# Gabrielcb/DaliID

Hardware: AMD Instinct MI355X
Metric: images/sec (train step) (higher is better)
Workload: dtype bf16; 1 GPU; configs[1]: ResNet-50 ReID bf16 256x128, PK batch 16x16=256 per GPU, center+proxy heads, Adam, EMA; global_batch=256, per_gpu_batch=256, parallelism=dp1

## Files before the change

daliid_amd/csrc/conv.hip:

```cpp
#include "gemm_tile.h"
#include "kernels.h"
#include "../../include/daliid_debug.h"
#include <cstdlib>
#include <type_traits>
#include <vector>
#include <string>
#include <cstdio>

namespace dali {

__device__ __forceinline__ void decode_pixel(const GatherGeom& g, int p, int& n, int& ho, int& wo) {
    if (g.lhw >= 0 && g.lw >= 0) {
        n = p >> g.lhw;
        const int rem = p & ((1 << g.lhw) - 1);
        ho = rem >> g.lw;
        wo = rem & ((1 << g.lw) - 1);
    } else {
        const int hw = g.Hout * g.Wout;
        n = p / hw;
        const int rem = p - n * hw;
        ho = rem / g.Wout;
        wo = rem - ho * g.Wout;
    }
}
// ... 1336 lines not shown
        if (ksteps > 1) dma_wait<4>(); else dma_wait<0>();
        __builtin_amdgcn_s_barrier();
        conv_stamp(a, 1);
        int st_cur = 0, st_nxt2 = 2;
        for (int kt = 0; kt < ksteps; ++kt) {
            if (kt + 2 < ksteps) issue(kt + 2, st_nxt2);
            const uint16_t* sa = smem + st_cur * 2 * TILE;
            const uint16_t* sb = sa + TILE;
            bf16x8_t fa[4];
            wgrad_tr_kstep(sa, wm * 4, sb, wn * 4, lane, acc, fa);
            if constexpr (COLSUM) if (do_cs) {
#pragma unroll
                for (int i = 0; i < 4; ++i) cs[i] = __builtin_amdgcn_mfma_f32_16x16x32_bf16(fa[i], ones, cs[i], 0, 0, 0);
            }
            if (kt + 2 < ksteps) dma_wait<4>(); else dma_wait<0>();
            __builtin_amdgcn_s_barrier();
            st_cur = (st_cur == 2) ? 0 : st_cur + 1;
            st_nxt2 = (st_nxt2 == 2) ? 0 : st_nxt2 + 1;
        }
    }
    conv_stamp(a, 2);
    float* slab = a.partial + (size_t)ks * a.Cm * a.Ntot;
    store_slab_tiles<4, 4>(slab, acc, m0 + wm * 64, n0 + wn * 64, a.Cm, a.Ntot, lane);
    if constexpr (COLSUM) if (do_cs && (lane & 15) == 0) {
#pragma unroll
        for (int i = 0; i < 4; ++i)
#pragma unroll
            for (int rr = 0; rr < 4; ++rr) {
                const int m = m0 + wm * 64 + i * 16 + (lane >> 4) * 4 + rr;
                if (m < a.Cm) a.colsum[(size_t)ks * a.Cm + m] = cs[i][rr];
            }
    }
    conv_stamp_stores(a);
}

__device__ __forceinline__ int halo_swz(int row) { return ((row >> 1) & 1) | (((row >> 3) & 1) << 1); }
constexpr int W3_A_ELEMS = 32 * 128, W3_B_ELEMS = 16 * 512, W3_STAGE = W3_A_ELEMS + W3_B_ELEMS;

template <int NSTAGE>
__global__ __launch_bounds__(512) void igemm_wgrad3x3_kernel(WGradArgs a, int tiles_m, int tiles_n) {
    extern __shared__ __attribute__((aligned(16))) uint16_t smem[];
    const int tid = threadIdx.x, lane = tid & 63;
    const int wave = __builtin_amdgcn_readfirstlane(tid >> 6);
    const int wm = wave >> 2, wn = wave & 3;
    WGradWork wk;
    if (!wk.map_xcd(a, tiles_m, tiles_n)) return;
    const int ks = wk.ks, m0 = wk.tm * 128, ci0 = wk.tn * 64;
    conv_stamp(a, 0);
    const bool m_active = m0 + wm * 64 < a.Cm;
    const GatherGeom g = a.g;
    const int W = g.Wout, H = g.Hout, Cin = g.Ck, lw = g.lw, lhw = g.lhw;
    const int RW = 32 >> lw, HC = W + 2, HP = (RW + 2) * HC;
    const WGradRsrc rs = wgrad_rsrc(a);

    const int r_in = lane >> 4, ps = lane & 15;
    const int c16 = ((((ps >> 1) ^ wg_swz(4 * wave + r_in)) << 1) | (ps & 1));
    const int am = m0 + c16 * 8;
    const bool a_ok = am < a.Cm;
    int hb_hr[2], hb_off[2];
    bool hb_ok[2];
#pragma unroll
    for (int i = 0; i < 2; ++i) {
        const int hp = 8 * (wave + 8 * i) + (lane >> 3);
        const int lc = (lane & 7) ^ (halo_swz(hp) << 1);
        const int hr = hp / HC, hc = hp - hr * HC;
        hb_hr[i] = hr;
// ... 562 lines not shown
    K64_CLS = ring_kernel<64, 4, 4, 4, 4, 2, 4, true, Epi::PARITY>("K64_CLS"),
    K64_SRC2 = ring_kernel<64, 4, 4, 4, 4, 2, 4, true, Epi::CONV, true>("K64_SRC2"),
    K64_FUSED_SRC2 = ring_kernel<64, 4, 4, 4, 4, 2, 4, true, Epi::FUSED, true>("K64_FUSED_SRC2"),
    K64_320 = ring_kernel<64, 4, 4, 4, 5, 2, 4, true, Epi::LIN>("K64_320");

template <int RB, bool RES, bool OM, bool BITS, bool SRC2 = false>
static GemmKernel f1_kernel() {
    static char name[32];
    snprintf(name, sizeof name, "F1_RB%d%s%s%s%s", RB, RES ? "_RES" : "", OM ? "_MASK" : "", BITS ? "_BITS" : "", SRC2 ? "_SRC2" : "");
    return {name, kfn(&fused1x1_persist_kernel<3, RB, RES, OM, BITS, SRC2>), (F1_NC + F1_NP + F1_NR) * 64, f1_lds_bytes(3, RB, RB == 2 ? 128 : F1_KMAX),
            F1_TM, F1_TN, GRID_CUS, 0, RB};
}
static const GemmKernel F1[2][2][2][2] = {
    {{{f1_kernel<2, false, false, false, true>(), f1_kernel<2, false, false, true>()}, {f1_kernel<2, false, true, false>(), f1_kernel<2, false, true, true>()}},
     {{f1_kernel<2, true, false, false>(), f1_kernel<2, true, false, true>()}, {f1_kernel<2, true, true, false>(), f1_kernel<2, true, true, true>()}}},
    {{{f1_kernel<1, false, false, false, true>(), f1_kernel<1, false, false, true>()}, {f1_kernel<1, false, true, false>(), f1_kernel<1, false, true, true>()}},
     {{f1_kernel<1, true, false, false>(), f1_kernel<1, true, false, true>()}, {f1_kernel<1, true, true, false>(), f1_kernel<1, true, true, true>()}}}};

static const GemmKernel
    WG_BN{"WG_BN", kfn(&igemm_wgrad_kernel<true>), 256, 0, 128, 128, GRID_SPLITS},
    WG_PLAIN{"WG_PLAIN", kfn(&igemm_wgrad_kernel<false>), 256, 0, 128, 128, GRID_SPLITS},
    WG_3X3{"WG_3X3", kfn(&igemm_wgrad3x3_kernel<3>), 512, 3 * W3_STAGE * 2, 128, 9 * 64, GRID_SPLITS8, 256};
static const GemmKernel WG_DMA[2] = {
    {"WG_DMA", kfn(&igemm_wgrad_dma_kernel<false>), 256, 0, 128, 128, GRID_SPLITS8},
    {"WG_DMA_COLSUM", kfn(&igemm_wgrad_dma_kernel<true>), 256, 0, 128, 128, GRID_SPLITS8}};
static const GemmKernel WG_WG[2] = {
    {"WG_WG", kfn(&igemm_wgrad_wg_kernel<2, 4, 3>), 512, ring_lds(128, 256, 32, 3), 128, 256, GRID_SPLITS8, 512},
    {"WG_WG_COLSUM", kfn(&igemm_wgrad_wg_kernel<2, 4, 3, true>), 512, ring_lds(128, 256, 32, 3), 128, 256, GRID_SPLITS8, 512}};
static const GemmKernel WG_P[2][2] = {
    {{"WG_P", kfn(&igemm_wgrad_p_kernel<2, 4, 4, 4, 8, 6>), 1024, ring_lds(128, 256, 32, 6), 128, 256, GRID_SPLITS8, 256},
     {"WG_P_COLSUM", kfn(&igemm_wgrad_p_kernel<2, 4, 4, 4, 8, 6, true>), 1024, ring_lds(128, 256, 32, 6), 128, 256, GRID_SPLITS8, 256}},
    {{"WG_P_FLAT", kfn(&igemm_wgrad_p_kernel<1, 4, 8, 4, 4, 6>), 512, ring_lds(128, 256, 32, 6), 128, 256, GRID_SPLITS8, 256},
     {"WG_P_FLAT_COLSUM", kfn(&igemm_wgrad_p_kernel<1, 4, 8, 4, 4, 6, true>), 512, ring_lds(128, 256, 32, 6), 128, 256, GRID_SPLITS8, 256}}};

struct GemmChoice {
    const GemmKernel* k = nullptr;
    int tiles_m = 0, tiles_n = 0, lds = 0, class_grid = 0;
    unsigned grid = 0;
    int rc = DALI_OK, why_arg = 0;
    const char* why = nullptr;
    GemmChoice() = default;
    GemmChoice(int rc_, const char* why_, int why_arg_ = 0) : rc(rc_), why_arg(why_arg_), why(why_) {}
    int refuse() const { set_error(why, why_arg); return rc; }
};
static GemmChoice gemm_place(const GemmKernel& k, int rows, int cols, int mult, int Ck) {
    GemmChoice c;
    c.k = &k;
    c.tiles_m = (rows + k.tm - 1) / k.tm;
    c.tiles_n = (cols + k.tn - 1) / k.tn;
    c.lds = k.f1_rb ? f1_lds_bytes(3, k.f1_rb, Ck) : k.lds;
    switch (k.grid) {
        case GRID_XCD: c.grid = xcd_tile_grid(c.tiles_m, c.tiles_n); break;
        case GRID_CLASSES: c.class_grid = xcd_tile_grid(c.tiles_m, c.tiles_n); c.grid = mult * c.class_grid; break;
        case GRID_CUS: c.grid = mult; break;
        case GRID_HALO: c.grid = c.tiles_n; break;
        case GRID_SPLITS: c.grid = c.tiles_m * c.tiles_n * mult; break;
        case GRID_SPLITS8: c.grid = (c.tiles_m * c.tiles_n * mult + 7) / 8 * 8; break;
    }
    return c;
}
template <class Args>
static int gemm_launch(hipStream_t st, const GemmChoice& c, Args& args) {
    const GemmKernel& k = *c.k;
    DeviceOnce::Guard once(k.once);
    if (k.lds > 64 * 1024 && once.first()) {
        DALI_HIP(hipFuncSetAttribute(k.fn, hipFuncAttributeMaxDynamicSharedMemorySize, k.lds));
// ... 232 lines not shown
    wgrad_plan(Cm, w.Ntot, P, 512, &w.splits, &w.pix_per_split, taps, halo_w);
    const int cfg = wgrad_pick_cfg(Cm, w.Ntot, taps, P, halo_w);
    const bool dma_ok = gather_dma_ok(g, P, (long long)P * Cm * 2);
    const bool colsum = want_colsum && wgrad_colsum_ok(cfg, in_bn, dma_ok);
    w.c = gemm_place(wgrad_kernel(cfg, Cm, w.Ntot, in_bn, dma_ok, colsum, plain_rows(g)), Cm, w.Ntot, w.splits, g.Ck);
    w.colsum_rows = colsum ? colsum_rows_of(*w.c.k, w.Ntot, w.splits) : 0;
    return w;
}

WGradNeed wgrad_need(int Cm, int P, const GatherGeom& g, bool colsum, bool operand_transform) {
    const WGradChoice w = wgrad_choose(Cm, P, g, operand_transform, colsum);
    return WGradNeed{(size_t)w.splits * Cm * w.Ntot * sizeof(float), colsum ? std::max((size_t)w.colsum_rows * Cm, colsum_partial_floats(P, Cm)) : 0};
}

int launch_wgrad(hipStream_t st, WGradArgs a, const WGradBufs& ws, float* out, int accumulate, float* colsum_out) {
    const WGradChoice w = wgrad_choose(a.Cm, a.P, a.g, a.in_scale != nullptr, colsum_out != nullptr);
    a.Ntot = w.Ntot; a.splits = w.splits; a.pix_per_split = w.pix_per_split;
    a.partial = ws.slab;
    a.colsum = w.colsum_rows ? ws.cs_partial : nullptr;
    a.stamps = g_conv_stamps;
    a.g.lw = ilog2_exact(a.g.Wout);
    a.g.lhw = ilog2_exact(a.g.Hout * a.g.Wout);
    {
    char what[160] = "";
    if (g_prof)
        snprintf(what, sizeof what, "wgrad,Cm=%d,K=%d,P=%d,taps=%d,stride=%d,sub=0,fused=%d,stats=0,res=0,mask=0,lin=%d", a.Cm, a.Ntot, a.P, a.g.R * a.g.S, a.g.stride,
                 a.in_scale ? 1 : 0, a.colsum ? 1 : 0);
    ProfScope prof_scope(st, 1, 2.0 * a.Cm * (double)a.Ntot * a.P, what);
    if (int rc = gemm_launch(st, w.c, a)) return rc;
    }
    if (int rc = launch_splitk_reduce2(st, a.partial, out, (size_t)a.Cm * a.Ntot, a.splits, accumulate, a.colsum, colsum_out, (size_t)a.Cm, w.colsum_rows)) return rc;
    if (!colsum_out || a.colsum) return DALI_OK;
    return launch_colsum(st, a.dY, a.P, a.Cm, colsum_out, ws.cs_partial, ws.scratch);
}

int launch_splitk_reduce(hipStream_t st, const float* partial, float* out, size_t elems, int splits, int accumulate) {
    return launch_splitk_reduce2(st, partial, out, elems, splits, accumulate, nullptr, nullptr, 0, 0);
}
int launch_splitk_reduce2(hipStream_t st, const float* partial, float* out, size_t elems, int splits, int accumulate,
                          const float* partial2, float* out2, size_t elems2, int splits2) {
    const size_t chunks = (elems + 3) / 4;
    const unsigned rblocks = (unsigned)((chunks + 63) / 64);
    const int W = splits >= 32 ? 16 : (splits >= 2 ? 4 : 1);
    const bool second = partial2 && out2 && elems2 > 0;
    if (second && ((elems & 3) || (elems2 & 3))) {
        if (int rc = launch_splitk_reduce2(st, partial, out, elems, splits, accumulate, nullptr, nullptr, 0, 0)) return rc;
        return launch_splitk_reduce2(st, partial2, out2, elems2, splits2, 0, nullptr, nullptr, 0, 0);
    }
    if (elems & 3) {
        hipLaunchKernelGGL(splitk_reduce_odd_kernel, dim3((unsigned)((elems + 255) / 256)), dim3(256), 0, st, partial, out, elems, splits, accumulate, W);
        DALI_LAUNCH_CHECK();
        return DALI_OK;
    }
    ReduceJob2 j2{nullptr, nullptr, 0, 0, 0xffffffffu};
    unsigned grid = rblocks;
    if (second) { j2 = ReduceJob2{partial2, out2, elems2, splits2, rblocks}; grid += (unsigned)((elems2 / 4 + 63) / 64); }
    switch (W) {
        case 1: hipLaunchKernelGGL(splitk_reduce_kernel<1>, dim3(grid), dim3(64), 0, st, partial, out, elems, splits, accumulate, j2); break;
        case 4: hipLaunchKernelGGL(splitk_reduce_kernel<4>, dim3(grid), dim3(256), 0, st, partial, out, elems, splits, accumulate, j2); break;
        default: hipLaunchKernelGGL(splitk_reduce_kernel<16>, dim3(grid), dim3(1024), 0, st, partial, out, elems, splits, accumulate, j2); break;
    }
    DALI_LAUNCH_CHECK();
    return DALI_OK;
}

}
// ... 214 lines not shown
}

extern "C" int dali_linear_fwd(dali_ctx* ctx, void* stream, const uint16_t* x, const uint16_t* w, const float* bias, int act,
                               const uint16_t* residual, uint16_t* y, uint16_t* pre, int rows, int K, int N) {
    DALI_REQUIRE(ctx && x && w && y, "dali_linear_fwd: null argument");
    DALI_REQUIRE(K % 32 == 0 && N % 4 == 0 && rows > 0, "dali_linear_fwd: K must be a multiple of 32 and N of 4 (K=%d N=%d)", K, N);
    DALI_REQUIRE(act == 0 || act == 1, "dali_linear_fwd: act must be 0 (none) or 1 (gelu)");
    return launch_linear_fwd((hipStream_t)stream, x, w, bias, act, residual, y, pre, nullptr, rows, K, N);
}
extern "C" int dali_linear_fwd_scaled(dali_ctx* ctx, void* stream, const uint16_t* x, const uint16_t* w, const float* bias, int act,
                                      const uint16_t* residual, const float* row_scale, uint16_t* y, int rows, int K, int N) {
    DALI_REQUIRE(ctx && x && w && y && row_scale, "dali_linear_fwd_scaled: null argument");
    DALI_REQUIRE(K % 32 == 0 && N % 4 == 0 && rows > 0, "dali_linear_fwd_scaled: K must be a multiple of 32 and N of 4 (K=%d N=%d)", K, N);
    DALI_REQUIRE(act == 0 || act == 1, "dali_linear_fwd_scaled: act must be 0 (none) or 1 (gelu)");
    return launch_linear_fwd((hipStream_t)stream, x, w, bias, act, residual, y, nullptr, nullptr, rows, K, N, row_scale);
}
extern "C" int dali_linear_dgrad(dali_ctx* ctx, void* stream, const uint16_t* dy, const uint16_t* wt, const uint16_t* gelu_pre,
                                 const uint16_t* residual, uint16_t* dx, int rows, int K, int N) {
    DALI_REQUIRE(ctx && dy && wt && dx, "dali_linear_dgrad: null argument");
    DALI_REQUIRE(N % 32 == 0 && K % 4 == 0 && rows > 0, "dali_linear_dgrad: N must be a multiple of 32 and K of 4 (K=%d N=%d)", K, N);
    return launch_linear_fwd((hipStream_t)stream, dy, wt, nullptr, 0, residual, dx, nullptr, gelu_pre, rows, N, K);
}
extern "C" int dali_linear_wgrad(dali_ctx* ctx, void* stream, const uint16_t* x, const uint16_t* dy, float* dw, float* dbias, int rows,
                                 int K, int N) {
    DALI_REQUIRE(ctx && x && dy && dw, "dali_linear_wgrad: null argument");
    DALI_REQUIRE(K % 8 == 0 && N % 8 == 0 && rows > 0, "dali_linear_wgrad: K and N must be multiples of 8");
    const WGradNeed need = linear_wgrad_need(rows, K, N, dbias != nullptr);
    const size_t slab = align_up(need.slab_bytes, 256), part = align_up(need.colsum_floats * 4, 256);
    char* ws = static_cast<char*>(workspace(ctx, slab + part + reduce_scratch_bytes(N, 1)));
    if (!ws) return DALI_ERR_NOMEM;
    const WGradBufs bufs{reinterpret_cast<float*>(ws), reinterpret_cast<float*>(ws + slab), reinterpret_cast<double*>(ws + slab + part)};
    return launch_linear_wgrad((hipStream_t)stream, x, dy, dw, rows, K, N, bufs, dbias);
}
```

daliid_amd/csrc/kernels.h:

```cpp
#pragma once
#include "common.h"

namespace dali {

struct GatherGeom {
    int Hout, Wout;
    int Hin, Win;
    int Ck;
    int R, S, stride, pad;
    int mode;
    long long img_pitch;
    int row_pitch, pix_pitch;
    int lw, lhw;
    int sub, oph, opw, Hfull, Wfull;
    int r0, rstep, nr, s0, sstep, ns;
    int class_grid;
};

struct IGemmArgs {
    const uint16_t* W;
    const uint16_t* X;
    uint16_t* O;
    const uint16_t* Res;
    const uint8_t* res_mask;
// ... 16 lines not shown
    const uint8_t* out_mask;
    const uint16_t* X2;
    int Ck1;
    int x_rep;
};

struct WGradArgs {
    const uint16_t* dY;
    const uint16_t* X;
    float* partial;
    const float* in_scale; const float* in_shift;
    int Cm, P, Ntot, in_relu;
    int splits, pix_per_split;
    GatherGeom g;
    unsigned long long* stamps;
    float* colsum;
};


struct TransposeJob { const uint16_t* w; uint16_t* wt; int Co, T, Ci, first_block; };
int launch_weight_transpose_batched(hipStream_t st, const TransposeJob* jobs, int n);

struct BnBwdSide { const uint16_t* raw; const float* mean; const float* invstd; const float* scale; const float* shift; };

int launch_igemm_conv(hipStream_t st, const IGemmArgs& a);
int gemm_profile_begin(hipStream_t st, int cls, double flops, const char* what);
void gemm_profile_end(hipStream_t st, int slot);
int igemm_conv_stat_tiles(int Cm, int P, int K, bool operand_transform = false);
bool conv_cat_act_supported(int Cm, int c1, int c2, int P, int parts = 1);
struct WGradNeed { size_t slab_bytes, colsum_floats; };
WGradNeed wgrad_need(int Cm, int P, const GatherGeom& g, bool colsum, bool operand_transform = false);
struct WGradBufs { float* slab; float* cs_partial; double* scratch; };
int launch_wgrad(hipStream_t st, WGradArgs a, const WGradBufs& ws, float* out, int accumulate, float* colsum_out = nullptr);
int launch_splitk_reduce2(hipStream_t st, const float* partial, float* out, size_t elems, int splits, int accumulate,
                          const float* partial2, float* out2, size_t elems2, int splits2);
int launch_splitk_reduce(hipStream_t st, const float* partial, float* out, size_t elems, int splits, int accumulate);

int launch_linear_fwd(hipStream_t st, const uint16_t* x, const uint16_t* w, const float* bias, int act, const uint16_t* residual, uint16_t* y,
                      uint16_t* pre, const uint16_t* dact_pre, int rows, int K, int N, const float* row_scale = nullptr);
int launch_linear_wgrad(hipStream_t st, const uint16_t* x, const uint16_t* dy, float* dw, int rows, int K, int N, const WGradBufs& ws, float* dbias = nullptr);
WGradNeed linear_wgrad_need(int rows, int K, int N, bool bias);

int launch_bnlin_stats(hipStream_t st, const uint16_t* W, const uint16_t* Wt, const float* gram, const float* m2, int C, int w, double count, const float* gamma,
                       const float* beta, float* rm, float* rv, float momentum, float eps, float* ut, float* dot, float* scale, float* shift,
                       float* mean, float* invstd);
int launch_bnlin_ut(hipStream_t st, const uint16_t* W, const float* gram, int C, int w, float* ut);
int launch_bnlin_bwd(hipStream_t st, const uint16_t* W, const uint16_t* Wt, const float* ut, const float* m2, const float* s_dz, int C,
                     int w, double count, const float* scale, const float* mean, const float* invstd, float* dW, float* dgamma, float* dbeta,
                     uint16_t* wd1, uint16_t* wd2, float* bvec, float* qk, int ld1 = 0, int ld2 = 0);

constexpr int REDUCE_SMAX = 64;
inline size_t reduce_scratch_bytes(int C, int NV) { return (size_t)REDUCE_SMAX * C * NV * sizeof(double); }
int launch_bn_finalize(hipStream_t st, const float* partial, int tiles, int C, double count, const float* gamma, const float* beta,
                       float* rm, float* rv, float momentum, float eps, float* scale, float* shift, float* mean, float* invstd,
                       double* scratch);
struct BnEvalJob { const float *gamma, *beta, *rm, *rv; float *scale, *shift; int C; };
struct BnEvalJobs { static constexpr int MAX = 56; BnEvalJob job[MAX]; };
int launch_bn_eval_coeffs_batched(hipStream_t st, const BnEvalJob* jobs, int n, float eps);
int launch_fold_cat_weights(hipStream_t st, const float* w3, const float* wd, const float* s3, const float* sd, const float* h3, const float* hd, int C, int w,
                            int cin, int parts, uint16_t* wcat, float* shcat);
int launch_bn_act(hipStream_t st, const uint16_t* raw, const float* scale, const float* shift, const uint16_t* idn, const uint16_t* raw2,
                  const float* scale2, const float* shift2, int relu, size_t elems, int C, uint16_t* y, uint8_t* mask_out);
int bn_bwd_blocks(int P, int C, int* rows_per_block);
size_t bn_bwd_partial_floats(int P, int C, bool dual);
int launch_bn_bwd(hipStream_t st, const uint16_t* g, const uint16_t* ymask, const uint8_t* ybits, const BnBwdSide& a, const BnBwdSide* b, int relu, int P, int C,
                  float* partial, float* coef_a, float* coef_b, float* dgamma_a, float* dbeta_a, float* dgamma_b, float* dbeta_b,
// ... 66 lines not shown
```

daliid_amd/csrc/resnet_plan.hip:

```cpp
#include "kernels.h"
#include "plan_table.h"
#include <cstring>
#include <new>

using namespace dali;

namespace {

struct Conv {
    int cin, cout, r, s, stride, pad, hin, win, hout, wout;
    int64_t w_off;
    uint16_t* w_bf16;
    uint16_t* wt_bf16;
};
struct Bn {
    int C;
    int64_t g_off, b_off;
    int64_t rm_off, rv_off;
    float *scale, *shift, *mean, *invstd, *coef;
};
struct LinBn {
    int w = 0, C = 0;
    bool stats = false;
    float *gram = nullptr, *m2 = nullptr, *bvec = nullptr, *qk = nullptr;
// ... 141 lines not shown
                add_conv(net, b.cd, pre + ".downsample.0", inpl, planes * 4, 1, st, 0, h, w);
                add_bn(net, b.bd, pre + ".downsample.1", planes * 4);
            }
            b.hout = b.c2.hout; b.wout = b.c2.wout;
            b.lin_ds = b.has_ds && st == 1 && inpl % 32 == 0 && inpl <= 128 && net->blocks.empty();
            h = b.hout; w = b.wout; inpl = planes * 4;
            net->blocks.push_back(b);
        }
        net->stage_last[li] = (int)net->blocks.size() - 1;
    }
    net->feat_dim = inpl;
    net->head_hw = h * w;
    DALI_REQUIRE(net->head_hw < 32768, "dali_resnet_create: final map too large");
    add_bn(net, net->neck, "last_bn", net->feat_dim);

    const size_t N = net->N;
    net->reserve(net->wbf16_flat, (size_t)net->param_elems * 2);
    net->reserve(net->w_stem, (size_t)wb * 224 * 2);
    net->reserve(net->ximg, N * (net->H + 6) * (net->W + 8) * 4 * 2);
    const size_t raw0_bytes = N * net->stem_h * net->stem_w * wb * 2;
    net->reserve(net->raw0, raw0_bytes);
    net->reserve(net->pool0, N * net->pool_h * net->pool_w * wb * 2);
    net->reserve(net->pool_arg, N * net->pool_h * net->pool_w * wb);
    reserve_bn(net, net->stem_bn);
    size_t max_act = raw0_bytes, max_stat = (size_t)igemm_conv_stat_tiles(wb, (int)N * net->stem_h * net->stem_w, 224) * wb * 2 * 4;
    int stem_qpb;
    size_t max_bwd_partial = (size_t)maxpool_bn_bwd_blocks((int)N, net->stem_h, net->stem_w, wb, &stem_qpb) * wb * 2 * 4;
    size_t max_slab = 0, max_cs = 256;
    auto size_wgrad = [&](const WGradDesc& d, bool colsum) {
        const WGradNeed need = wgrad_need(d.Cm, d.P, d.g, colsum);
        max_slab = std::max(max_slab, need.slab_bytes);
        max_cs = std::max(max_cs, need.colsum_floats * 4);
    };
    size_wgrad(stem_wgrad_desc(net), false);
    for (auto& b : net->blocks) {
        const size_t pin = N * b.hin * b.win, pout = N * b.hout * b.wout;
        net->reserve(b.raw1, pin * b.width * 2);
        net->reserve(b.a1, pin * b.width * 2);
        net->reserve(b.raw2, pout * b.width * 2);
        net->reserve(b.a2, pout * b.width * 2);
        reserve_linbn(net, b.l3, b.c3, true);
        net->reserve(b.sdz, (size_t)b.cout * 4);
        size_wgrad(gram_desc(net, b.c3), true);
        net->reserve(b.y, pout * b.cout * 2);
        net->reserve(b.ybits, pout * b.cout / 8);
        if (b.has_ds) net->reserve(b.rawd, pout * b.cout * 2);
        if (b.lin_ds) {
            reserve_linbn(net, b.ld, b.cd, false);
            size_wgrad(gram_desc(net, b.cd), true);
        }
        b.cat_eval = b.has_ds && b.cd.stride == 1 && conv_cat_act_supported(b.cout, b.width, b.cin, (int)pout, 2);
        if (b.cat_eval) { net->reserve(b.wcat, (size_t)b.cout * 2 * (b.width + b.cin) * 2); net->reserve(b.shcat, (size_t)b.cout * 4); }
        for_each_bn(b, [&](Bn& bn) { reserve_bn(net, bn); });
        for_each_conv(b, [&](Conv& c) {
            net->reserve(c.wt_bf16, (size_t)c.cin * c.r * c.s * c.cout * 2);
            const int P = (int)N * c.hout * c.wout;
            max_stat = std::max(max_stat, (size_t)igemm_conv_stat_tiles(c.cout, P, c.r * c.s * c.cin) * c.cout * 2 * 4);
            size_wgrad(conv_wgrad_desc(net, c), &c == &b.c3);
            max_act = std::max(max_act, (size_t)P * c.cout * 2);
            max_act = std::max(max_act, N * c.hin * c.win * c.cin * 2);
            max_bwd_partial = std::max(max_bwd_partial, bn_bwd_partial_floats(P, c.cout, true) * 4);
        });
    }
    net->reserve(net->feat, N * net->feat_dim * 4);
    net->reserve(net->dfeat, N * net->feat_dim * 4);
    net->reserve(net->head_arg, N * net->feat_dim * 2);
    net->reserve(net->neck_mean, net->feat_dim * 4);
    net->reserve(net->neck_invstd, net->feat_dim * 4);
    net->reserve(net->stat_partial, max_stat);
    net->reserve(net->bwd_partial, max_bwd_partial);
    net->reserve(net->wgrad_slab, max_slab);
    net->reserve(net->cs_partial, max_cs);
    net->reserve(net->stem_dw_pad, (size_t)wb * 224 * 4);
    net->reserve(net->red_scratch, reduce_scratch_bytes(net->feat_dim, 3));
    net->gbuf_bytes = align_up(max_act, 256);
    for (int i = 0; i < 6; ++i) net->reserve(net->gbuf[i], net->gbuf_bytes);
    *out = net;
    return DALI_OK;
}

extern "C" int dali_resnet_destroy(dali_resnet* net) { delete net; return DALI_OK; }

// ... 72 lines not shown
    a.out_scale = bn.scale; a.out_shift = bn.shift; a.out_relu = 1;
    a.Cm = c.cout; a.P = net->N * c.hout * c.wout;
    a.g = conv_geom(c, 0);
    return launch_igemm_conv(st, a);
}

int conv_wgrad(dali_resnet* net, hipStream_t st, const Conv& c, const uint16_t* x, const uint16_t* dy) {
    return run_wgrad(net, st, conv_wgrad_desc(net, c), dy, x, net->G + c.w_off);
}

int conv_dgrad(dali_resnet* net, hipStream_t st, const Conv& c, const uint16_t* dy, const uint16_t* residual, uint16_t* dx,
               const uint8_t* out_mask = nullptr) {
    IGemmArgs a{};
    a.W = c.wt_bf16; a.X = dy; a.O = dx; a.Res = residual; a.out_mask = out_mask;
    a.Cm = c.cin; a.P = net->N * c.hin * c.win;
    a.g = conv_geom(c, 1);
    return launch_igemm_conv(st, a);
}

int cat_gemm(dali_resnet* net, hipStream_t st, const Conv& c, int mode, const uint16_t* W, const uint16_t* X, int c1, const uint16_t* X2, int c2, int Cm,
             uint16_t* O, IGemmArgs stage = IGemmArgs{}) {
    IGemmArgs& a = stage;
    a.W = W; a.X = X; a.X2 = X2; a.Ck1 = c1; a.O = O;
    a.Cm = Cm; a.P = net->N * (mode == 0 ? c.hout * c.wout : c.hin * c.win);
    Conv cat = c;
    (mode == 0 ? cat.cin : cat.cout) = (a.x_rep ? a.x_rep : 1) * (c1 + c2);
    a.g = conv_geom(cat, mode);
    return launch_igemm_conv(st, a);
}

int linbn_fwd(dali_resnet* net, hipStream_t st, LinBn& l, const Conv& c, Bn& bn, const uint16_t* x) {
    const WGradDesc d = gram_desc(net, c);
    int rc;
    if ((rc = run_wgrad(net, st, d, x, x, l.gram, l.m2))) return rc;
    if (!l.stats) return launch_bnlin_ut(st, c.w_bf16, l.gram, l.C, l.w, l.ut);
    const BnParams p = bn_params(net, bn);
    return launch_bnlin_stats(st, c.w_bf16, c.wt_bf16, l.gram, l.m2, l.C, l.w, (double)d.P, p.gamma, p.beta, p.rm, p.rv, 0.1f, 1e-5f, l.ut, l.dot, bn.scale,
                              bn.shift, bn.mean, bn.invstd);
}
int linbn_bwd(dali_resnet* net, hipStream_t st, LinBn& l, const Conv& c, const Bn& bn, const uint16_t* dz, const uint16_t* x, float* s_dz, bool sum_dz) {
    const WGradDesc d = conv_wgrad_desc(net, c);
    int rc;
    if ((rc = run_wgrad(net, st, d, dz, x, net->G + c.w_off, sum_dz ? s_dz : nullptr))) return rc;
    const int ld = l.C + l.w;
    return launch_bnlin_bwd(st, c.w_bf16, c.wt_bf16, l.ut, l.m2, s_dz, l.C, l.w, (double)d.P, bn.scale, bn.mean, bn.invstd, net->G + c.w_off, net->G + bn.g_off,
                            net->G + bn.b_off, l.wd, l.wd + l.C, l.bvec, l.qk, ld, ld);
}

int bn_bwd(dali_resnet* net, hipStream_t st, const Bn& bn, const uint16_t* raw, const uint16_t* g, int relu, int P, uint16_t* out) {
    const BnBwdSide s{raw, bn.mean, bn.invstd, bn.scale, bn.shift};
    return launch_bn_bwd(st, g, nullptr, nullptr, s, nullptr, relu, P, bn.C, net->bwd_partial, bn.coef, nullptr, net->G + bn.g_off, net->G + bn.b_off,
                         nullptr, nullptr, out, nullptr, nullptr, net->red_scratch);
}

uint16_t* next_gbuf(dali_resnet* net, const uint16_t* avoid0, const uint16_t* avoid1 = nullptr, const uint16_t* avoid2 = nullptr,
                    const uint16_t* avoid3 = nullptr) {
    for (int i = 0; i < 6; ++i) {
        uint16_t* g = net->gbuf[i];
        if (g != avoid0 && g != avoid1 && g != avoid2 && g != avoid3) return g;
    }
    return nullptr;
}

int stem_forward(dali_resnet* net, hipStream_t st, const float* images, bool tr) {
    const Conv& c = net->stem;
    Bn& bn = net->stem_bn;
    int rc;
// ... 269 lines not shown
```

include/daliid_debug.h:

```cpp
#ifndef DALIID_DEBUG_H
#define DALIID_DEBUG_H

#include <stdint.h>

#ifdef __cplusplus
extern "C" {
#endif

int dali_debug_reload_env(void);

int dali_debug_set_conv_stamps(void* dev_ptr);

int dali_debug_wgrad_splits(int Cm, int Ntot, int P, int taps, int halo_w);

enum {
    DALI_DEBUG_CONV_STATS = 1,
    DALI_DEBUG_CONV_FUSED = 2,
    DALI_DEBUG_CONV_RES = 4,
    DALI_DEBUG_CONV_RES_MASK = 8,
    DALI_DEBUG_CONV_OUT_MASK = 16,
    DALI_DEBUG_CONV_BITS = 32,
    DALI_DEBUG_CONV_LIN = 64
};
int dali_debug_conv_kernel_name(int Cm, int P, int h, int wd, int ck, int r, int s, int stride, int pad, int mode, int flags, int ck1, int x_rep,
                                int n_cus, char* out, int cap);

int dali_debug_splitk_reduce(void* stream, const float* partial, float* out, long long elems, int splits, int accumulate);

struct dali_resnet;
int dali_debug_resnet_backward_block(struct dali_resnet* net, void* stream, const float* d_emb, int block);

struct dali_vit;
int dali_debug_vit_backward_block(struct dali_vit* net, void* stream, const float* d_feat, int block);
int dali_debug_vit_tensor(const struct dali_vit* net, const char* name, void** ptr, int64_t* bytes);

struct dali_ctx;
int dali_debug_stem_wgrad(struct dali_ctx* ctx, void* stream, const float* images, const unsigned short* d_raw0, int N, int H, int W, int Cout, float* dw);
int dali_debug_head_pool_bwd_masked(struct dali_ctx* ctx, void* stream, const float* df, const short* arg, int n, int hw, int C, int mode,
                                    const unsigned char* ybits, unsigned short* dx);

#ifdef __cplusplus
}
#endif
#endif
```

Before: 17810 images/s.

## Add dedicated symmetric Gram kernel for linear-BN statistics with fold for width 64

Introduces a specialized X^T X Gram kernel with DMA-to-LDS ring buffering that computes only upper-triangular tiles and mirrors them, and folds pairs of rows into a 128-wide k-step for width 64. For width 64, four waves' partial results are reduced through LDS. It also computes column sums via MFMA with a ones vector. The default PLAN path only uses the new kernel when width is 64; other widths fall back to the generic wgrad path. The aim is to avoid redundant symmetric work and underused tiles on narrow Gram computations, at the cost of extra code paths and workspace sizing changes.

```diff
diff --git a/daliid_amd/csrc/conv.hip b/daliid_amd/csrc/conv.hip
--- a/daliid_amd/csrc/conv.hip
+++ b/daliid_amd/csrc/conv.hip
@@ -1392,6 +1392,162 @@
             }
     }
     conv_stamp_stores(a);
+}
+
+template <int N, int K>
+__device__ __forceinline__ void gram_dma_wait(int k) {
+    if constexpr (K == 0) dma_wait<0>();
+    else {
+        if (k >= K) dma_wait<K * N>();
+        else gram_dma_wait<N, K - 1>(k);
+    }
+}
+
+template <bool FOLD, int NIMG, int NSTAGE>
+__global__ __launch_bounds__(256) void igemm_gram_kernel(WGradArgs a, int tiles_m, int tiles_n) {
+    constexpr int IMG = 32 * 128, STAGE = NIMG * IMG, AHEAD = NSTAGE - 1;
+    constexpr int KROWS = FOLD ? 64 : 32;
+    static_assert(!FOLD || (NIMG == 2 && NSTAGE * STAGE * 2 >= 4 * 64 * 64 * 4), "FOLD: two row groups per k-step; the ring holds the four wave results");
+    extern __shared__ __attribute__((aligned(16))) uint16_t smem[];
+    const int tid = threadIdx.x, lane = tid & 63;
+    const int wave = __builtin_amdgcn_readfirstlane(tid >> 6);
+    WGradWork wk;
+    if (!wk.map_xcd(a, tiles_m, tiles_n)) return;
+    const int w = a.Cm, ks = wk.ks;
+    int ti = 0, tj = wk.tm;
+    if constexpr (!FOLD) {
+        const int nt = (w + 127) >> 7;
+        while (tj >= nt - ti) { tj -= nt - ti; ++ti; }
+        tj += ti;
+    }
+    const bool diag = ti == tj;
+    const int nimg = (FOLD || !diag) ? 2 : 1;
+    const int row_begin = FOLD ? wk.p_begin >> 1 : wk.p_begin, row_end = FOLD ? (wk.p_end + 1) >> 1 : wk.p_end;
+    const int ksteps = row_end > row_begin ? (row_end - row_begin + KROWS - 1) / KROWS : 0;
+    const int row_w = FOLD ? 128 : w;
+    const __amdgpu_buffer_rsrc_t rs = wgrad_rsrc(a).y;
+
+    const int r_in = lane >> 4, ps = lane & 15;
+    const int c16 = ((((ps >> 1) ^ wg_swz(4 * wave + r_in)) << 1) | (ps & 1));
+    int col[2];
+    bool col_ok[2];
+    col[0] = (FOLD ? 0 : ti * 128) + c16 * 8; col[1] = (FOLD ? 0 : tj * 128) + c16 * 8;
+    col_ok[0] = col[0] < row_w; col_ok[1] = col[1] < row_w;
+
+    auto issue = [&](int kt, int stage) {
+        uint16_t* base = smem + stage * STAGE;
+#pragma unroll
+        for (int img = 0; img < NIMG; ++img) {
+            if (img < nimg) {
+#pragma unroll
+                for (int i = 0; i < 2; ++i) {
+                    const int blk = wave + 4 * i;
+                    const int row = row_begin + kt * KROWS + (FOLD ? img * 32 : 0) + 4 * blk + r_in;
+                    const uint32_t off = (row < row_end && col_ok[img]) ? (uint32_t)(row * row_w + col[img]) * 2u : DMA_OOB;
+                    __builtin_amdgcn_raw_ptr_buffer_load_lds(rs, (lds_void_ptr)(base + img * IMG + blk * 512), 16, off, 0, 0, 0);
+                }
+            }
+        }
+    };
+    auto wait_steps = [&](int k) {
+        if constexpr (NIMG == 2) {
+            if (nimg == 2) gram_dma_wait<4, AHEAD - 1>(k);
+            else gram_dma_wait<2, AHEAD - 1>(k);
+        } else gram_dma_wait<2, AHEAD - 1>(k);
+    };
+
+    const int wm = FOLD ? (wave & 1) : (wave >> 1), wn = wave & 1;
+    const int img_a = FOLD ? (wave >> 1) : 0, img_b = FOLD ? (wave >> 1) : (diag ? 0 : 1);
+    const bool active = FOLD || !diag || wm <= wn;
+    const bool do_cs = FOLD || (diag && wm == wn);
+
+    f32x4_t acc[4][4];
+#pragma unroll
+    for (int i = 0; i < 4; ++i)
+#pragma unroll
+        for (int j = 0; j < 4; ++j) acc[i][j] = f32x4_t{0.f, 0.f, 0.f, 0.f};
+    f32x4_t cs[4];
+#pragma unroll
+    for (int i = 0; i < 4; ++i) cs[i] = f32x4_t{0.f, 0.f, 0.f, 0.f};
+    typedef short ones_vec_t __attribute__((ext_vector_type(8)));
+    const bf16x8_t ones = __builtin_bit_cast(bf16x8_t, ones_vec_t{0x3F80, 0x3F80, 0x3F80, 0x3F80, 0x3F80, 0x3F80, 0x3F80, 0x3F80});
+
+    if (ksteps > 0) {
+        int issued = 0;
+        for (; issued < AHEAD && issued < ksteps; ++issued) issue(issued, issued);
+        wait_steps(issued - 1);
+        __builtin_amdgcn_s_barrier();
+        int st_cur = 0, st_fill = AHEAD;
+        for (int kt = 0; kt < ksteps; ++kt) {
+            if (kt + AHEAD < ksteps) issue(kt + AHEAD, st_fill);
+            if (active) {
+                const uint16_t* sa = smem + st_cur * STAGE + img_a * IMG;
+                const uint16_t* sb = smem + st_cur * STAGE + img_b * IMG;
+                bf16x8_t fa[4];
+                wgrad_tr_kstep(sa, wm * 4, sb, wn * 4, lane, acc, fa);
+                if (do_cs) {
+#pragma unroll
+                    for (int i = 0; i < 4; ++i) cs[i] = __builtin_amdgcn_mfma_f32_16x16x32_bf16(fa[i], ones, cs[i], 0, 0, 0);
+                }
+            }
+            const int left = ksteps - 1 - kt;
+            wait_steps((left < AHEAD ? left : AHEAD) - 1);
+            __builtin_amdgcn_s_barrier();
+            st_cur = (st_cur == NSTAGE - 1) ? 0 : st_cur + 1;
+            st_fill = (st_fill == NSTAGE - 1) ? 0 : st_fill + 1;
+        }
+    }
+    float* slab = a.partial + (size_t)ks * w * w;
+    if constexpr (FOLD) {
+        float* red = reinterpret_cast<float*>(smem);
+#pragma unroll
+        for (int i = 0; i < 4; ++i)
+#pragma unroll
+            for (int j = 0; j < 4; ++j)
+#pragma unroll
+                for (int rr = 0; rr < 4; ++rr) red[((wave * 16 + i * 4 + j) * 4 + rr) * 64 + lane] = acc[i][j][rr];
+        __syncthreads();
+        f32x4_t sum[1][4];
+#pragma unroll
+        for (int j = 0; j < 4; ++j)
+#pragma unroll
+            for (int rr = 0; rr < 4; ++rr) {
+                float s = red[((0 * 16 + wave * 4 + j) * 4 + rr) * 64 + lane];
+#pragma unroll
+                for (int v = 1; v < 4; ++v) s += red[((v * 16 + wave * 4 + j) * 4 + rr) * 64 + lane];
+                sum[0][j][rr] = s;
+            }
+        store_slab_tiles<1, 4>(slab, sum, wave * 16, 0, w, w, lane);
+        if ((lane & 15) == 0) {
+#pragma unroll
+            for (int i = 0; i < 4; ++i)
+#pragma unroll
+                for (int rr = 0; rr < 4; ++rr) a.colsum[((size_t)ks * 4 + wave) * w + i * 16 + (lane >> 4) * 4 + rr] = cs[i][rr];
+        }
+    } else {
+        if (!active) return;
+        const int m_first = ti * 128 + wm * 64, n_first = tj * 128 + wn * 64;
+        store_slab_tiles<4, 4>(slab, acc, m_first, n_first, w, w, lane);
+        if (!diag || wm != wn) {
+            const int mc = m_first + (lane >> 4) * 4, nr = n_first + (lane & 15);
+#pragma unroll
+            for (int i = 0; i < 4; ++i)
+#pragma unroll
+                for (int j = 0; j < 4; ++j) {
+                    const int m = mc + i * 16, n = nr + j * 16;
+                    if (m < w && n < w) *reinterpret_cast<f32x4_t*>(slab + (size_t)n * w + m) = acc[i][j];
+                }
+        }
+        if (do_cs && (lane & 15) == 0) {
+#pragma unroll
+            for (int i = 0; i < 4; ++i)
+#pragma unroll
+                for (int rr = 0; rr < 4; ++rr) {
+                    const int m = m_first + i * 16 + (lane >> 4) * 4 + rr;
+                    if (m < w) a.colsum[(size_t)ks * w + m] = cs[i][rr];
+                }
+        }
+    }
 }
 
 __device__ __forceinline__ int halo_swz(int row) { return ((row >> 1) & 1) | (((row >> 3) & 1) << 1); }
@@ -2020,6 +2176,10 @@
      {"WG_P_COLSUM", kfn(&igemm_wgrad_p_kernel<2, 4, 4, 4, 8, 6, true>), 1024, ring_lds(128, 256, 32, 6), 128, 256, GRID_SPLITS8, 256}},
     {{"WG_P_FLAT", kfn(&igemm_wgrad_p_kernel<1, 4, 8, 4, 4, 6>), 512, ring_lds(128, 256, 32, 6), 128, 256, GRID_SPLITS8, 256},
      {"WG_P_FLAT_COLSUM", kfn(&igemm_wgrad_p_kernel<1, 4, 8, 4, 4, 6, true>), 512, ring_lds(128, 256, 32, 6), 128, 256, GRID_SPLITS8, 256}}};
+static const GemmKernel WG_GRAM[3] = {
+    {"WG_GRAM_FOLD", kfn(&igemm_gram_kernel<true, 2, 4>), 256, 4 * 2 * 8192, 128, 128, GRID_SPLITS8},
+    {"WG_GRAM_ONE", kfn(&igemm_gram_kernel<false, 1, 8>), 256, 8 * 8192, 128, 128, GRID_SPLITS8},
+    {"WG_GRAM", kfn(&igemm_gram_kernel<false, 2, 4>), 256, 4 * 2 * 8192, 128, 128, GRID_SPLITS8}};
 
 struct GemmChoice {
     const GemmKernel* k = nullptr;
@@ -2318,6 +2478,55 @@
     if (int rc = launch_splitk_reduce2(st, a.partial, out, (size_t)a.Cm * a.Ntot, a.splits, accumulate, a.colsum, colsum_out, (size_t)a.Cm, w.colsum_rows)) return rc;
     if (!colsum_out || a.colsum) return DALI_OK;
     return launch_colsum(st, a.dY, a.P, a.Cm, colsum_out, ws.cs_partial, ws.scratch);
+}
+
+static int g_gram_force_splits = 0;
+static bool gram_takes(int w, int P, const GatherGeom& g) {
+    return plain_rows(g) && g.Ck == w && w % 64 == 0 && w >= 64 && w <= 512 && P > 0 && dma_addressable((long long)P * w * 2);
+}
+static bool gram_pays(int w) { return w == 64; }
+static bool gram_on_kernel(GramPath path, int w, int P, const GatherGeom& g) {
+    return path != GramPath::GENERIC && gram_takes(w, P, g) && (path == GramPath::KERNEL || gram_pays(w));
+}
+static int gram_kstep_pixels(int w) { return w == 64 ? 128 : 32; }
+struct GramChoice { int splits, pix_per_split, colsum_rows; GemmChoice c; };
+static GramChoice gram_choose(int w, int P) {
+    GramChoice gc{};
+    const int nt = (w + 127) / 128, tiles = w == 64 ? 1 : nt * (nt + 1) / 2, kpix = gram_kstep_pixels(w);
+    const int ksteps = (P + kpix - 1) / kpix;
+    int sp = g_gram_force_splits > 0 ? g_gram_force_splits : std::min(std::max(256 / tiles, 1), std::max(ksteps / 16, 1));
+    sp = std::min(sp, ksteps);
+    const int pps = ((P + sp - 1) / sp + kpix - 1) / kpix * kpix;
+    gc.splits = (P + pps - 1) / pps;
+    gc.pix_per_split = pps;
+    gc.colsum_rows = w == 64 ? 4 * gc.splits : gc.splits;
+    const GemmKernel& k = WG_GRAM[w == 64 ? 0 : (w == 128 ? 1 : 2)];
+    gc.c.k = &k;
+    gc.c.tiles_m = tiles; gc.c.tiles_n = 1; gc.c.lds = k.lds;
+    gc.c.grid = (unsigned)((tiles * gc.splits + 7) / 8 * 8);
+    return gc;
+}
+WGradNeed gram_need(int w, int P, const GatherGeom& g, GramPath path) {
+    if (!gram_on_kernel(path, w, P, g)) return wgrad_need(w, P, g, true);
+    const GramChoice gc = gram_choose(w, P);
+    return WGradNeed{(size_t)gc.splits * w * w * sizeof(float), (size_t)gc.colsum_rows * w};
+}
+int launch_gram(hipStream_t st, const uint16_t* x, int P, int w, const GatherGeom& g, const WGradBufs& ws, float* gram, float* m2, GramPath path) {
+    WGradArgs a{};
+    a.dY = x; a.X = x; a.Cm = w; a.P = P; a.g = g;
+    if (!gram_on_kernel(path, w, P, g)) return launch_wgrad(st, a, ws, gram, 0, m2);
+    const GramChoice gc = gram_choose(w, P);
+    a.Ntot = w; a.splits = gc.splits; a.pix_per_split = gc.pix_per_split;
+    a.partial = ws.slab; a.colsum = ws.cs_partial;
+    a.g.lw = ilog2_exact(a.g.Wout);
+    a.g.lhw = ilog2_exact(a.g.Hout * a.g.Wout);
+    {
+    char what[160] = "";
+    if (g_prof) snprintf(what, sizeof what, "wgrad,Cm=%d,K=%d,P=%d,taps=1,stride=1,sub=0,fused=0,stats=0,res=0,mask=0,lin=1", w, w, P);
+    ProfScope prof_scope(st, 1, 2.0 * w * (double)w * P, what);
+    if (int rc = gemm_launch(st, gc.c, a)) return rc;
+    }
+    return launch_splitk_reduce2(st, a.partial, gram, (size_t)w * w, a.splits, 0, a.colsum, m2, (size_t)w, gc.colsum_rows);
 }
 
 int launch_splitk_reduce(hipStream_t st, const float* partial, float* out, size_t elems, int splits, int accumulate) {
@@ -2598,3 +2807,42 @@
     const WGradBufs bufs{reinterpret_cast<float*>(ws), reinterpret_cast<float*>(ws + slab), reinterpret_cast<double*>(ws + slab + part)};
     return launch_linear_wgrad((hipStream_t)stream, x, dy, dw, rows, K, N, bufs, dbias);
 }
+
+extern "C" int dali_debug_gram(dali_ctx* ctx, void* stream, const uint16_t* x, int P, int w, int flags, float* gram, float* m2) {
+    DALI_REQUIRE(ctx && x && gram && m2, "dali_debug_gram: null argument");
+    DALI_REQUIRE(P > 0 && w > 0 && w % 8 == 0, "dali_debug_gram: w must be a multiple of 8 (P=%d w=%d)", P, w);
+    const GramPath path = (flags & 1) ? GramPath::GENERIC : GramPath::KERNEL;
+    GatherGeom g{};
+    linear_geom(g, w);
+    g_gram_force_splits = flags >> 8;
+    const WGradNeed need = gram_need(w, P, g, path);
+    const size_t slab = align_up(need.slab_bytes, 256), part = align_up(need.colsum_floats * 4, 256);
+    char* ws = static_cast<char*>(workspace(ctx, slab + part + reduce_scratch_bytes(w, 1)));
+    int rc = DALI_ERR_NOMEM;
+    if (ws) {
+        const WGradBufs bufs{reinterpret_cast<float*>(ws), reinterpret_cast<float*>(ws + slab), reinterpret_cast<double*>(ws + slab + part)};
+        rc = launch_gram((hipStream_t)stream, x, P, w, g, bufs, gram, m2, path);
+    }
+    g_gram_force_splits = 0;
+    return rc;
+}
+extern "C" int dali_debug_gram_plan(int w, int P, int* splits, int* pix_per_split, int* kstep_pixels, long long* slab_bytes, long long* colsum_floats) {
+    GatherGeom g{};
+    linear_geom(g, w);
+    const bool takes = gram_takes(w, P, g);
+    const WGradNeed need = gram_need(w, P, g, GramPath::KERNEL);
+    if (takes) {
+        const GramChoice gc = gram_choose(w, P);
+        if (splits) *splits = gc.splits;
+        if (pix_per_split) *pix_per_split = gc.pix_per_split;
+        if (kstep_pixels) *kstep_pixels = gram_kstep_pixels(w);
+    } else {
+        const WGradChoice wc = wgrad_choose(w, P, g, false, true);
+        if (splits) *splits = wc.splits;
+        if (pix_per_split) *pix_per_split = wc.pix_per_split;
+        if (kstep_pixels) *kstep_pixels = 32;
+    }
+    if (slab_bytes) *slab_bytes = (long long)need.slab_bytes;
+    if (colsum_floats) *colsum_floats = (long long)need.colsum_floats;
+    return (takes ? 1 : 0) | (gram_on_kernel(GramPath::PLAN, w, P, g) ? 2 : 0);
+}
diff --git a/daliid_amd/csrc/kernels.h b/daliid_amd/csrc/kernels.h
--- a/daliid_amd/csrc/kernels.h
+++ b/daliid_amd/csrc/kernels.h
@@ -72,6 +72,10 @@
 WGradNeed wgrad_need(int Cm, int P, const GatherGeom& g, bool colsum, bool operand_transform = false);
 struct WGradBufs { float* slab; float* cs_partial; double* scratch; };
 int launch_wgrad(hipStream_t st, WGradArgs a, const WGradBufs& ws, float* out, int accumulate, float* colsum_out = nullptr);
+enum class GramPath { PLAN, GENERIC, KERNEL };
+WGradNeed gram_need(int w, int P, const GatherGeom& g, GramPath path = GramPath::PLAN);
+int launch_gram(hipStream_t st, const uint16_t* x, int P, int w, const GatherGeom& g, const WGradBufs& ws, float* gram, float* m2,
+                GramPath path = GramPath::PLAN);
 int launch_splitk_reduce2(hipStream_t st, const float* partial, float* out, size_t elems, int splits, int accumulate,
                           const float* partial2, float* out2, size_t elems2, int splits2);
 int launch_splitk_reduce(hipStream_t st, const float* partial, float* out, size_t elems, int splits, int accumulate);
diff --git a/daliid_amd/csrc/resnet_plan.hip b/daliid_amd/csrc/resnet_plan.hip
--- a/daliid_amd/csrc/resnet_plan.hip
+++ b/daliid_amd/csrc/resnet_plan.hip
@@ -197,6 +197,11 @@
         max_slab = std::max(max_slab, need.slab_bytes);
         max_cs = std::max(max_cs, need.colsum_floats * 4);
     };
+    auto size_gram = [&](const WGradDesc& d) {
+        const WGradNeed need = gram_need(d.Cm, d.P, d.g);
+        max_slab = std::max(max_slab, need.slab_bytes);
+        max_cs = std::max(max_cs, need.colsum_floats * 4);
+    };
     size_wgrad(stem_wgrad_desc(net), false);
     for (auto& b : net->blocks) {
         const size_t pin = N * b.hin * b.win, pout = N * b.hout * b.wout;
@@ -206,13 +211,13 @@
         net->reserve(b.a2, pout * b.width * 2);
         reserve_linbn(net, b.l3, b.c3, true);
         net->reserve(b.sdz, (size_t)b.cout * 4);
-        size_wgrad(gram_desc(net, b.c3), true);
+        size_gram(gram_desc(net, b.c3));
         net->reserve(b.y, pout * b.cout * 2);
         net->reserve(b.ybits, pout * b.cout / 8);
         if (b.has_ds) net->reserve(b.rawd, pout * b.cout * 2);
         if (b.lin_ds) {
             reserve_linbn(net, b.ld, b.cd, false);
-            size_wgrad(gram_desc(net, b.cd), true);
+            size_gram(gram_desc(net, b.cd));
         }
         b.cat_eval = b.has_ds && b.cd.stride == 1 && conv_cat_act_supported(b.cout, b.width, b.cin, (int)pout, 2);
         if (b.cat_eval) { net->reserve(b.wcat, (size_t)b.cout * 2 * (b.width + b.cin) * 2); net->reserve(b.shcat, (size_t)b.cout * 4); }
@@ -351,7 +356,7 @@
 int linbn_fwd(dali_resnet* net, hipStream_t st, LinBn& l, const Conv& c, Bn& bn, const uint16_t* x) {
     const WGradDesc d = gram_desc(net, c);
     int rc;
-    if ((rc = run_wgrad(net, st, d, x, x, l.gram, l.m2))) return rc;
+    if ((rc = launch_gram(st, x, d.P, d.Cm, d.g, WGradBufs{net->wgrad_slab, net->cs_partial, net->red_scratch}, l.gram, l.m2))) return rc;
     if (!l.stats) return launch_bnlin_ut(st, c.w_bf16, l.gram, l.C, l.w, l.ut);
     const BnParams p = bn_params(net, bn);
     return launch_bnlin_stats(st, c.w_bf16, c.wt_bf16, l.gram, l.m2, l.C, l.w, (double)d.P, p.gamma, p.beta, p.rm, p.rv, 0.1f, 1e-5f, l.ut, l.dot, bn.scale,
diff --git a/include/daliid_debug.h b/include/daliid_debug.h
--- a/include/daliid_debug.h
+++ b/include/daliid_debug.h
@@ -27,6 +27,11 @@
 
 int dali_debug_splitk_reduce(void* stream, const float* partial, float* out, long long elems, int splits, int accumulate);
 
+struct dali_ctx;
+enum { DALI_DEBUG_GRAM_GENERIC = 1 };
+int dali_debug_gram(struct dali_ctx* ctx, void* stream, const unsigned short* x, int P, int w, int flags, float* gram, float* m2);
+int dali_debug_gram_plan(int w, int P, int* splits, int* pix_per_split, int* kstep_pixels, long long* slab_bytes, long long* colsum_floats);
+
 struct dali_resnet;
 int dali_debug_resnet_backward_block(struct dali_resnet* net, void* stream, const float* d_emb, int block);
 
```

Result: no change. 17860 images/s, median of 6 (+0.3%).
